# MobilePerceptionLab/EventCalib

Hardware: AMD Instinct MI355X
Metric: Mevents/s DBSCAN+detect (higher is better)
Workload: dtype f64; 1 GPU; ONE 50M-event synthetic circle-grid stream (BASELINE configs[2]'s stream), 346x260, 1 Mev/s, tiled 1.5 ms windows (33334 windows), eps 4 minpts 2; stages: window bounds + EventFrame slicing (reference point order) + DBSCAN(+/-) + circle candidates (reference tie picks); HBM-resident when the timed region starts, upload excluded (reported beside: h2d, ingest); events_total=50000000, events_covered_by_the_ranks_windows=50000000, windows_total=33334, events_per_gpu=50000000, windows_per_gpu=33334, unique_points_per_gpu=38558159, max_window_events=1501, max_segment_points=666, windows_reaching_pairing=26228, circle_candidates=839094, event_point=False

## Files before the change

eventcalib_amd/csrc/extract_window.hpp:

```cpp
#pragma once
#include "ecal_ctx.hpp"
#include "block_utils.hpp"
#include "ref_nth_element.hpp"
#include <type_traits>

#pragma clang fp contract(off)

namespace ecal {

#ifdef ECAL_PHASE_PROF
static __device__ unsigned long long g_det_cycles[16];
#define DET_MARK(idx)                                                                    \
    do {                                                                                 \
        if (threadIdx.x == 0) {                                                          \
            const unsigned long long now__ = __builtin_readcyclecounter();               \
            atomicAdd(&g_det_cycles[idx], now__ - det_t__);                              \
            det_t__ = now__;                                                             \
        }                                                                                \
    } while (0)
#define DET_T0() unsigned long long det_t__ = __builtin_readcyclecounter()
#else
#define DET_MARK(idx) do { } while (0)
#define DET_T0() do { } while (0)
#endif
#ifndef ECAL_DET_STOP
#define ECAL_DET_STOP 0
#endif

constexpr int DET_T = 256;
constexpr uint32_t DET_MAXC = 2048;
constexpr uint32_t DET_LDS_PTS = 1408;
constexpr uint32_t DET_LDS_MAXC = 384;
constexpr uint32_t DET_LDS_PTS2 = 2816, DET_LDS_MAXC2 = 512;

struct DetectParams {
    uint32_t cluster_min;
    uint32_t need_clusters;
    double four_thr2;
    double thr;
    uint32_t fit_circle;
    uint32_t knn;
    const uint32_t *xy16;
    const uint32_t *seg_fmt;
    const uint32_t *px_tree = nullptr, *px_tree_flag = nullptr;
    uint32_t px_tree_epoch = 0;
    int tie_e2i = 0, tie_prune = 0;
};
constexpr uint32_t DET_TIE_TREE_CAP = 768;
constexpr size_t DET_TIE_INV_BYTES = DET_TIE_TREE_CAP;
constexpr uint32_t DET_KNN_MAX = 8;

__device__ __forceinline__ double norm_of(double2 p) { return __dsqrt_rn(p.x * p.x + p.y * p.y); }

struct DetGlobal {
    const double2 *pts;
    uint32_t *members, *sorted, *koff, *ksize, *rep;
    int32_t *kept;
    double *norms;
    __device__ __forceinline__ double2 pt(uint32_t li) const { return pts[li]; }
    __device__ __forceinline__ double norm(uint32_t li) const { return norms[li]; }
    __device__ __forceinline__ double key(uint32_t li) const { return norms[li]; }
    __device__ __forceinline__ void set_norm(uint32_t li, double v) const { norms[li] = v; }
    static constexpr bool INT_PIXELS = false;
    static constexpr uint32_t REP_TIE = 0x80000000u;
    static constexpr uint32_t REP_BAD = 0x40000000u;
    static constexpr uint32_t IDX_MASK = 0xFFFFFFFFu, IDXB = 0u;
    static constexpr int J = 1;
    static constexpr uint32_t MAXC = 0;
    using CIdx = uint32_t;
    static constexpr CIdx CNONE = 0xFFFFFFFFu;
    __device__ __forceinline__ bool composite() const { return false; }
    __device__ __forceinline__ uint32_t member_word(uint32_t, uint32_t i) const { return i; }
    __device__ __forceinline__ uint32_t ipt(uint32_t) const { return 0; }
    __device__ __forceinline__ int32_t label(uint32_t, const int32_t *lab, uint32_t i) const { return lab[i]; }
};
template <uint32_t PTS_, uint32_t MAXC_>
struct DetLdsT {
    static constexpr uint32_t IDXB = PTS_ > 2048u ? 12u : 11u;
    static constexpr uint32_t IDX_MASK = (1u << IDXB) - 1u;
    static constexpr uint32_t REP_TIE = 0x8000u;
    static constexpr uint32_t REP_BAD = 0x4000u;
    static constexpr int J = (int) ((PTS_ + 255u) / 256u);
    static constexpr uint32_t MAXC = MAXC_;
    uint32_t *pts;
    uint32_t *members;
    uint16_t *sorted, *koff, *ksize, *rep;
    int16_t *kept;
    bool small;
    static constexpr bool INT_PIXELS = true;
    using CIdx = uint16_t;
    static constexpr CIdx CNONE = 0xFFFFu;
    __device__ __forceinline__ bool composite() const { return small; }
    __device__ __forceinline__ uint32_t member_word(uint32_t li, uint32_t i) const { return small ? (key(li) << IDXB) | i : i; }
    __device__ __forceinline__ uint32_t ipt(uint32_t li) const { return pts[li]; }
    __device__ __forceinline__ int32_t label(uint32_t li, const int32_t *, uint32_t) const { return kept[li]; }
    __device__ __forceinline__ double2 pt(uint32_t li) const {
        const uint32_t w = pts[li];
        return make_double2((double) (int) (short) (w & 0xFFFFu), (double) (((int) w) >> 16));
    }
    __device__ __forceinline__ double norm(uint32_t li) const { return norm_of(pt(li)); }
    __device__ __forceinline__ uint32_t key(uint32_t li) const {
        const uint32_t w = pts[li];
        const int x = (int) (short) (w & 0xFFFFu), y = ((int) w) >> 16;
        return (uint32_t) (x * x + y * y);
    }
    __device__ __forceinline__ void set_norm(uint32_t, double) const {}
};

struct CircleFit {
    double err, radius, cx, cy;
};

template <typename ST>
__device__ __forceinline__ CircleFit fit_pair(const ST &st, const uint32_t (&base)[2], const uint32_t (&kb)[2], uint32_t kp,
                                              uint32_t kn, double thr) {
    double sx = 0, sy = 0, sxx = 0, syy = 0, sxy = 0, sxxx = 0, syyy = 0, sxyy = 0, sxxy = 0;
    uint32_t cnt = 0;
    for (int pol = 0; pol < 2; pol++) {
        const uint32_t o = base[pol], kk = pol ? kn : kp;
        const uint32_t m = st.ksize[kb[pol] + kk], first = o + st.koff[kb[pol] + kk];
        for (uint32_t t = 0; t < m; t++) {
            const double2 e = st.pt(o + st.sorted[first + t]);
            sx += e.x;
            sy += e.y;
            const double xx = e.x * e.x, yy = e.y * e.y, xy = e.x * e.y;
            sxx += xx;
            syy += yy;
            sxy += xy;
            sxxx += xx * e.x;
            syyy += yy * e.y;
            sxyy += xy * e.y;
            sxxy += e.x * xy;
        }
        cnt += m;
    }
    double A[3][4] = {{2 * sx, 2 * sy, (double) cnt, sxx + syy},
                      {2 * sxx, 2 * sxy, sx, sxxx + sxyy},
                      {2 * sxy, 2 * syy, sy, sxxy + syyy}};
#pragma unroll
    for (int c = 0; c < 3; c++) {
        int piv = c;
#pragma unroll
        for (int r = c + 1; r < 3; r++)
            if (fabs(A[r][c]) > fabs(A[piv][c])) piv = r;
#pragma unroll
        for (int k = 0; k < 4; k++) {
            const double a = A[c][k], b = A[piv][k];
            A[c][k] = b;
            A[piv][k] = (piv == c) ? b : a;
        }
#pragma unroll
        for (int r = c + 1; r < 3; r++) {
            const double f = A[r][c] / A[c][c];
#pragma unroll
            for (int k = c; k < 4; k++) A[r][k] -= f * A[c][k];
        }
    }
    double x[3];
    x[2] = A[2][3] / A[2][2];
    x[1] = (A[1][3] - A[1][2] * x[2]) / A[1][1];
    x[0] = (A[0][3] - A[0][1] * x[1] - A[0][2] * x[2]) / A[0][0];
    CircleFit f;
    f.cx = x[0];
    f.cy = x[1];
    f.radius = __dsqrt_rn(x[0] * x[0] + x[1] * x[1] + x[2]);
    f.err = 0.0;
    const double2 pr = st.pt(base[0] + st.rep[kb[0] + kp]), nr = st.pt(base[1] + st.rep[kb[1] + kn]);
    const double ax = pr.x - nr.x, ay = pr.y - nr.y;
    const double approx = __dsqrt_rn(ax * ax + ay * ay) / 2;
    if (f.radius > thr || f.radius > 2 * approx) {
        f.err = 1.79769313486231570e308;
        return f;
    }
    for (int pol = 0; pol < 2; pol++) {
        const uint32_t o = base[pol], kk = pol ? kn : kp;
        const uint32_t m = st.ksize[kb[pol] + kk], first = o + st.koff[kb[pol] + kk];
        for (uint32_t t = 0; t < m; t++) {
            const double2 e = st.pt(o + st.sorted[first + t]);
            const double ex = e.x - f.cx, ey = e.y - f.cy;
            f.err += fabs(__dsqrt_rn(ex * ex + ey * ey) - f.radius);
        }
    }
    f.err /= (double) cnt * f.radius;
    return f;
}

template <typename ST>
__device__ __forceinline__ uint32_t knn_gated(const ST &st, uint32_t base_pol, uint32_t kb_pol, uint32_t nk, double2 q, uint32_t K,
                                              double gate, uint32_t (&idx)[DET_KNN_MAX]) {
    double d2[DET_KNN_MAX];
    for (uint32_t i = 0; i < DET_KNN_MAX; i++) {
        d2[i] = 1.79769313486231570e308;
        idx[i] = 0;
    }
    uint32_t have = 0;
    for (uint32_t k = 0; k < nk; k++) {
        const double2 c = st.pt(base_pol + st.rep[kb_pol + k]);
        const double dx = q.x - c.x, dy = q.y - c.y;
        const double d = dx * dx + dy * dy;
        uint32_t pos = have < K ? have : K;
        while (pos > 0 && d < d2[pos - 1]) pos--;
        if (pos < K) {
            for (uint32_t m = (have < K ? have : K - 1); m > pos; m--) {
                d2[m] = d2[m - 1];
                idx[m] = idx[m - 1];
            }
            d2[pos] = d;
            idx[pos] = k;
            if (have < K) have++;
        }
    }
    uint32_t real = K;
    for (uint32_t oi = 0; oi < K; oi++)
        if (d2[oi] > d2[0] * 4 || d2[oi] > gate) {
            real = oi;
            break;
        }
    return real;
}

template <typename ST>
__device__ __forceinline__ uint32_t ref_nth_member(const ST &st, uint32_t o, uint32_t *a, uint32_t m, uint32_t nth) {
    ecal::ref_nth_element(a, m, nth, [&](uint32_t x, uint32_t y) { return st.key(o + x) < st.key(o + y); });
    return a[nth];
}

struct LaneArr {
    using value_type = uint32_t;
    uint32_t *v;
    uint32_t off;
    struct Ref {
        uint32_t *v;
        uint32_t lane;
        __device__ __forceinline__ operator uint32_t() const { return (uint32_t) __builtin_amdgcn_readlane((int) *v, (int) lane); }
        __device__ __forceinline__ Ref &operator=(uint32_t x) {
            *v = (threadIdx.x & 63u) == lane ? x : *v;
            return *this;
        }
        __device__ __forceinline__ Ref &operator=(const Ref &o) { return *this = (uint32_t) o; }
    };
    __device__ __forceinline__ Ref operator[](int64_t i) const { return Ref{v, (uint32_t) __builtin_amdgcn_readfirstlane((int) (off + (uint32_t) i))}; }
    __device__ __forceinline__ LaneArr operator+(uint32_t d) const { return LaneArr{v, off + d}; }
};

template <typename ST>
__device__ __forceinline__ bool resolve_ties_inline(const ST &st, const uint32_t (&base)[2], const uint32_t (&kb)[2], const uint32_t (&n_pol)[2],
                                                    const uint32_t (&nk)[2], uint32_t tied0, uint32_t tied1, const uint32_t *tree_win,
                                                    int e2i, int prune, uint32_t *tree_lds, unsigned char *scratch,
                                                    uint8_t *inv, uint32_t *fail_word) {
    constexpr uint32_t WS = 1408, LIST_OFF = 200, LIST_BYTES = WS - LIST_OFF, NIL = 0xFFFFu;
    const uint32_t tid = threadIdx.x, lane = tid & 63u, wave = tid >> 6;
    unsigned char *const ws = scratch + wave * WS;
    uint8_t *const queue = ws + 128;
    uint32_t *const inq = reinterpret_cast<uint32_t *>(ws + 192);
    uint8_t *const lists = ws + LIST_OFF;
    if (tid == 0) *fail_word = 0;
    for (int pol = 0; pol < 2; pol++) {
        __syncthreads();
        if (!(pol ? tied1 : tied0)) continue;
        const uint32_t o = base[pol];
#ifdef ECAL_PHASE_PROF
        const unsigned long long tie_t0__ = __builtin_readcyclecounter();
#endif
        for (uint32_t i = tid; i < n_pol[pol]; i += DET_T) tree_lds[i] = tree_win[o + i];
        __syncthreads();
#ifdef ECAL_PHASE_PROF
        if (tid == 0) atomicAdd(&g_det_cycles[9], __builtin_readcyclecounter() - tie_t0__);
#endif
        for (uint32_t k = wave; k < nk[pol]; k += DET_T / 64) {
            const uint32_t rv = st.rep[kb[pol] + k];
            if (!(rv & ST::REP_TIE)) continue;
            const uint32_t m = st.ksize[kb[pol] + k], first = o + st.koff[kb[pol] + k];
            if (m > 64u || !st.composite()) {
                if (lane == 0) *fail_word = 1;
                continue;
            }
#ifdef ECAL_PHASE_PROF
            unsigned long long tie_t__ = __builtin_readcyclecounter();
#define TIE_MARK(i) do { if (lane == 0) { const unsigned long long n__ = __builtin_readcyclecounter(); atomicAdd(&g_det_cycles[i], n__ - tie_t__); tie_t__ = n__; } } while (0)
            if (lane == 0) {
                atomicAdd(&g_det_cycles[13], 1ull);
                atomicAdd(&g_det_cycles[14], (unsigned long long) m);
            }
#else
#define TIE_MARK(i) do { } while (0)
#endif
            const uint32_t slot = LIST_BYTES / m > 63u ? 63u : LIST_BYTES / m;
            const uint32_t p = lane < m ? st.sorted[first + lane] : 0u;
            if (lane < m) inv[p] = (uint8_t) lane;
            if (lane < 2u) inq[lane] = lane == 0 ? 1u : 0u;
            if (lane == 0) queue[0] = 0;
            __builtin_amdgcn_fence(__ATOMIC_RELEASE, "wavefront");
            __builtin_amdgcn_wave_barrier();
            const bool tiny = m <= 16u;
            unsigned long long hl = 0;
            uint32_t cnt = 0;
            bool bad = false;
            if (lane < m) {
                const uint32_t pw = st.ipt(o + p);
                const int qx = (int) (short) (pw & 0xFFFFu), qy = ((int) pw) >> 16;
                uint8_t *const out = lists + lane * slot;
                unsigned long long s0 = 0, s1 = 0, s2 = 0;
                uint32_t sp = 0, node = 0, dir = 0;
                for (;;) {
                    while (node != NIL) {
                        const uint32_t nw = st.ipt(o + node);
                        const int nx = (int) (short) (nw & 0xFFFFu), ny = ((int) nw) >> 16;
                        const int ddx = nx - qx, ddy = ny - qy;
                        if (ddx * ddx + ddy * ddy <= e2i && node != p && st.kept[o + node] == (int) k) {
                            if (tiny) hl |= (unsigned long long) inv[node] << (4u * cnt);
                            else if (cnt < slot) out[cnt] = inv[node];
                            cnt++;
                        }
                        const int dx = dir ? (qy - ny) : (qx - nx);
                        const uint32_t t = tree_lds[node], l = t & 0xFFFFu, r = t >> 16;
                        const uint32_t nearc = dx <= 0 ? l : r, farc = dx <= 0 ? r : l;
                        if ((dx < 0 ? -dx : dx) <= prune && farc != NIL) {
                            if (sp < 12u) {
                                s2 = (s2 << 16) | (s1 >> 48);
                                s1 = (s1 << 16) | (s0 >> 48);
                                s0 = (s0 << 16) | (farc | ((dir ^ 1u) << 15));
                            }
                            sp++;
                        }
                        node = nearc;
                        dir ^= 1u;
                    }
                    if (sp == 0 || sp > 12u) break;
                    sp--;
                    const uint32_t e = (uint32_t) (s0 & 0xFFFFu);
                    s0 = (s0 >> 16) | (s1 << 48);
                    s1 = (s1 >> 16) | (s2 << 48);
                    s2 >>= 16;
                    node = e & 0x7FFFu;
                    dir = e >> 15;
                }
                bad = (!tiny && cnt > slot) || sp > 12u;
            }
            __builtin_amdgcn_fence(__ATOMIC_RELEASE, "wavefront");
            __builtin_amdgcn_wave_barrier();
            TIE_MARK(10);
            uint32_t head = 0, tail = 1;
            const bool any_bad = __any(bad);
            unsigned long long qv = 0;
            if (tiny && !any_bad) {
                uint32_t inqm = 1u;
                while (head < tail) {
                    const int q = __builtin_amdgcn_readfirstlane((int) ((qv >> (4u * head)) & 15u));
                    head++;
                    const uint32_t lo = (uint32_t) __builtin_amdgcn_readlane((int) (uint32_t) hl, q);
                    const uint32_t hi = (uint32_t) __builtin_amdgcn_readlane((int) (uint32_t) (hl >> 32), q);
                    const unsigned long long hq = ((unsigned long long) hi << 32) | lo;
                    const uint32_t mq = (uint32_t) __builtin_amdgcn_readlane((int) cnt, q);
                    for (uint32_t t = mq; t-- > 0;) {
                        const uint32_t j = (uint32_t) (hq >> (4u * t)) & 15u;
                        if (!((inqm >> j) & 1u)) {
                            inqm |= 1u << j;
                            qv |= (unsigned long long) j << (4u * tail);
                            tail++;
                        }
                    }
                }
            }
            while (!tiny && !any_bad && head < tail) {
                const uint32_t q = reinterpret_cast<volatile uint8_t *>(queue)[head];
                head++;
                const uint32_t mq = (uint32_t) __shfl((int) cnt, (int) q, 64);
                bool take = false;
                uint32_t j = 0;
                if (lane < mq) {
                    j = lists[q * slot + (mq - 1u - lane)];
                    const uint32_t bit = 1u << (j & 31u);
                    take = !(atomicOr(&inq[j >> 5], bit) & bit);
                }
                const unsigned long long mask = __ballot(take);
                if (take) queue[tail + __popcll(mask & ((1ull << lane) - 1ull))] = (uint8_t) j;
                tail += (uint32_t) __popcll(mask);
                __builtin_amdgcn_fence(__ATOMIC_RELEASE, "wavefront");
                __builtin_amdgcn_wave_barrier();
            }
            if (any_bad || tail != m) {
                if (lane == 0) *fail_word = 1;
                continue;
            }
            TIE_MARK(11);
            uint32_t aw = 0;
            if (lane < m) {
                const uint32_t pid = st.sorted[first + (tiny ? (uint32_t) (qv >> (4u * lane)) & 15u : (uint32_t) queue[lane])];
                aw = st.member_word(o + pid, pid);
            }
            ecal::ref_nth_element(LaneArr{&aw, 0u}, m, m / 2u, [](uint32_t x, uint32_t y) { return (x >> ST::IDXB) < (y >> ST::IDXB); });
            const uint32_t pick = (uint32_t) __builtin_amdgcn_readlane((int) aw, (int) (m / 2u)) & ST::IDX_MASK;
            if (lane == 0)
                st.rep[kb[pol] + k] = (typename std::remove_reference<decltype(st.rep[0])>::type) (pick | ST::REP_TIE | ST::REP_BAD);
            TIE_MARK(12);
#undef TIE_MARK
        }
    }
    __syncthreads();
    return *fail_word == 0;
}

template <bool FIT, bool ORD, bool TDET, typename ST>
__device__ __forceinline__ void extract_window(const ST &st, const uint32_t (&base)[2], const uint32_t (&kb)[2],
                                               const uint32_t (&n_pol)[2], const int32_t *lab0, const int32_t *lab1,
                                               const int32_t *ord0, const int32_t *ord1, uint32_t *tie_list, uint32_t *tie_count,
                                               uint32_t tie_token, int32_t *mark0, int32_t *mark1,
                                               const uint32_t (&nc_pol)[2], const DetectParams &prm, uint32_t *csize,
                                               typename ST::CIdx *newid, typename ST::CIdx *coff,
                                               unsigned long long *red, uint32_t *nk_sh, uint32_t *info,
                                               uint32_t *cand_pair, double *cand_xyr, const uint32_t *tie_tree, const uint32_t *tie_flags,
                                               uint8_t *tie_inv) {
    const uint32_t tid = threadIdx.x;
    DET_T0();
    for (int pol = 0; pol < 2; pol++) {
        const uint32_t o = base[pol], ko = kb[pol], n = n_pol[pol], nc = nc_pol[pol];
        const int32_t *lab = pol ? lab1 : lab0;
        for (uint32_t c = tid; c < nc; c += DET_T) csize[c] = 0;
        __syncthreads();
        for (uint32_t i = tid; i < n; i += DET_T) {
            const int32_t l = st.label(o + i, lab, i);
            if (l >= 0) atomicAdd(&csize[l], 1u);
        }
        __syncthreads();
        {
            const uint32_t per = (nc + DET_T - 1) / DET_T, c0 = tid * per;
            uint32_t k = 0, m = 0;
            for (uint32_t c = c0; c < c0 + per && c < nc; c++) {
                if (csize[c] >= prm.cluster_min) {
                    k++;
                    m += csize[c];
                }
            }
            uint32_t ek, em, tk, tm;
            if constexpr (ST::INT_PIXELS) block_exscan_pair16<DET_T>(k, m, red, &ek, &em, &tk, &tm);
            else block_exscan_pair<DET_T>(k, m, red, &ek, &em, &tk, &tm);
            for (uint32_t c = c0; c < c0 + per && c < nc; c++) {
                if (csize[c] >= prm.cluster_min) {
                    newid[c] = (typename ST::CIdx) ek;
                    coff[c] = (typename ST::CIdx) em;
                    st.koff[ko + ek] = em;
                    st.ksize[ko + ek] = csize[c];
                    ek++;
                    em += csize[c];
                } else {
                    newid[c] = ST::CNONE;
                }
            }
            if (tid == 0) {
                nk_sh[pol] = tk;
                nk_sh[2 + pol] = tm;
            }
        }
        __syncthreads();
        for (uint32_t i = tid; i < n; i += DET_T) {
            const int32_t l = st.label(o + i, lab, i);
            int32_t kl = -1;
            if (l >= 0 && newid[l] != ST::CNONE) {
                kl = (int32_t) newid[l];
                const uint32_t at = atomicSub(&csize[l], 1u) - 1u;
                st.members[o + coff[l] + at] = st.member_word(o + i, i);
                st.set_norm(o + i, norm_of(st.pt(o + i)));
            }
            st.kept[o + i] = kl;
        }
        __syncthreads();
    }
    DET_MARK(1);
    if (ECAL_DET_STOP == 2) return;
    const uint32_t nk[2] = {nk_sh[0], nk_sh[1]};
    if (nk[0] < prm.need_clusters || nk[1] < prm.need_clusters) {
        if (tid == 0) {
            info[0] = 0;
            info[1] = nk[0];
            info[2] = nk[1];
            info[3] = 1;
        }
        return;
    }
    const uint32_t tm0 = nk_sh[2], tm1 = nk_sh[3];
    for (uint32_t idx = tid; idx < tm0 + tm1; idx += DET_T) {
        const int pol = idx >= tm0 ? 1 : 0;
        const uint32_t o = base[pol];
        const uint32_t wq = st.members[o + idx - (pol ? tm0 : 0u)];
        const uint32_t i = st.composite() ? (wq & ST::IDX_MASK) : wq;
        const int32_t kl = st.kept[o + i];
        const uint32_t m = st.ksize[kb[pol] + kl], first = o + st.koff[kb[pol] + kl];
        uint32_t rank = 0, at = 0, eq = 0;
        if (st.composite()) {
            const uint32_t wi = wq;
            for (uint32_t t = 0; t < m; t++) {
                const uint32_t wj = st.members[first + t];
                rank += (wj < wi) ? 1u : 0u;
                at += ((wj & ST::IDX_MASK) < i) ? 1u : 0u;
                if constexpr (ORD || TDET) eq += ((wj >> ST::IDXB) == (wi >> ST::IDXB)) ? 1u : 0u;
            }
        } else {
            const auto ni = st.key(o + i);
            for (uint32_t t = 0; t < m; t++) {
                const uint32_t j = st.members[first + t];
                const auto nj = st.key(o + j);
                rank += (nj < ni || (nj == ni && j < i)) ? 1u : 0u;
                at += (j < i) ? 1u : 0u;
                if constexpr (ORD || TDET) eq += (nj == ni) ? 1u : 0u;
            }
        }
        if (rank == m / 2) st.rep[kb[pol] + kl] = ((ORD || TDET) && eq > 1u) ? (i | ST::REP_TIE) : i;
        st.sorted[first + at] = i;
    }
    __syncthreads();
    if constexpr (TDET && !ORD) {
        for (int pol = 0; pol < 2; pol++)
            for (uint32_t k = tid; k < nk[pol]; k += DET_T)
                if (st.rep[kb[pol] + k] & ST::REP_TIE) nk_sh[pol] |= 0x80000000u;
        __syncthreads();
        const uint32_t tied0 = nk_sh[0] >> 31, tied1 = nk_sh[1] >> 31;
        const bool window_tied = (tied0 | tied1) != 0;
        __syncthreads();
        if (tid == 0) {
            nk_sh[0] &= 0x7FFFFFFFu;
            nk_sh[1] &= 0x7FFFFFFFu;
        }
        bool resolved = false;
        if constexpr (ST::INT_PIXELS) {
            if (window_tied && tie_tree) {
                constexpr bool FIRST_LAYOUT = ST::IDXB == 11u;
                constexpr uint32_t TREE_CAP = FIRST_LAYOUT ? DET_TIE_TREE_CAP : 1408u;
                static_assert(FIRST_LAYOUT ? 8u * ST::MAXC >= 4u * DET_TIE_TREE_CAP : 8u * ST::MAXC >= 1408u, "the tree / the positions fit where csize, newid and coff lay");
                uint32_t *const tree_lds = FIRST_LAYOUT ? csize : st.members + 1408;
                uint8_t *const inv = FIRST_LAYOUT ? tie_inv : reinterpret_cast<uint8_t *>(csize);
                const bool ok0 = !tied0 || (n_pol[0] <= TREE_CAP && tie_flags[0] == prm.px_tree_epoch);
                const bool ok1 = !tied1 || (n_pol[1] <= TREE_CAP && tie_flags[1] == prm.px_tree_epoch);
                if (ok0 && ok1 && inv)
                    resolved = resolve_ties_inline(st, base, kb, n_pol, nk, tied0, tied1, tie_tree, prm.tie_e2i, prm.tie_prune, tree_lds,
                                                   reinterpret_cast<unsigned char *>(st.members), inv, &nk_sh[2]);
            }
        }
        for (int pol = 0; pol < 2; pol++)
            for (uint32_t k = tid; k < nk[pol]; k += DET_T) {
                const uint32_t rv = st.rep[kb[pol] + k];
                if (!(rv & ST::REP_TIE)) continue;
                const uint32_t idx = rv & ~(ST::REP_TIE | ST::REP_BAD);
                if (resolved) {
                    st.rep[kb[pol] + k] = idx;
                } else {
                    st.rep[kb[pol] + k] = idx;
                    int32_t *mk = pol ? mark1 : mark0;
                    if (mk) mk[idx] = -3;
                }
            }
        __syncthreads();
        if (tid == 0 && window_tied && !resolved) {
            if (tie_list) tie_list[atomicAdd(tie_count, 1u)] = tie_token | ((tied0 ^ 1u) << 30) | ((tied1 ^ 1u) << 31);
        }
        __syncthreads();
        if (window_tied && !resolved && tie_list) return;
    }
    if constexpr (ORD) {
        if (tid == 0) nk_sh[2] = 0;
        for (int pol = 0; pol < 2; pol++) {
            const int32_t *ord = pol ? ord1 : ord0;
            for (uint32_t i = tid; i < n_pol[pol]; i += DET_T) {
                const int32_t kl = st.kept[base[pol] + i];
                if (kl < 0) continue;
                const uint32_t rv = st.rep[kb[pol] + kl];
                if (!(rv & ST::REP_TIE)) continue;
                const int32_t p = ord ? ord[i] : -1;
                if (p < 0 || (uint32_t) p >= st.ksize[kb[pol] + kl]) st.rep[kb[pol] + kl] = rv | ST::REP_BAD;
            }
        }
        __syncthreads();
        for (int pol = 0; pol < 2; pol++) {
            const int32_t *ord = pol ? ord1 : ord0;
            for (uint32_t i = tid; i < n_pol[pol]; i += DET_T) {
                const int32_t kl = st.kept[base[pol] + i];
                if (kl < 0) continue;
                const uint32_t rv = st.rep[kb[pol] + kl];
                if ((rv & (ST::REP_TIE | ST::REP_BAD)) != ST::REP_TIE) continue;
                st.members[base[pol] + st.koff[kb[pol] + kl] + (uint32_t) ord[i]] = i;
            }
        }
        __syncthreads();
        for (int pol = 0; pol < 2; pol++) {
            for (uint32_t k = tid; k < nk[pol]; k += DET_T) {
                const uint32_t rv = st.rep[kb[pol] + k];
                if (!(rv & ST::REP_TIE)) continue;
                uint32_t pick = rv & ~(ST::REP_TIE | ST::REP_BAD);
                const uint32_t m = st.ksize[kb[pol] + k], first = base[pol] + st.koff[kb[pol] + k];
                if (!(rv & ST::REP_BAD)) pick = ref_nth_member(st, base[pol], &st.members[first], m, m / 2u);
                else nk_sh[2] = 1;
                st.rep[kb[pol] + k] = pick;
            }
        }
        __syncthreads();
    }
    DET_MARK(2);
    if (ECAL_DET_STOP == 3) return;
    uint32_t carry = 0;
    auto emit = [&](uint32_t pi, bool ok, uint32_t ni_best, double cx, double cy, double r) {
        uint32_t ex, dummy, tot, dummy2;
        block_exscan_pair16<DET_T>(ok ? 1u : 0u, 0u, red, &ex, &dummy, &tot, &dummy2);
        if (ok) {
            const size_t at = (size_t) carry + ex;
            cand_pair[2 * at] = pi;
            cand_pair[2 * at + 1] = ni_best;
            cand_xyr[3 * at] = cx;
            cand_xyr[3 * at + 1] = cy;
            cand_xyr[3 * at + 2] = r;
        }
        carry += tot;
    };
    bool paired = false;
    if constexpr (!FIT && ST::INT_PIXELS) {
        if (st.composite() && nk[0] <= 64u && nk[1] <= 64u) {
            paired = true;
            static_assert(4 * ST::MAXC >= 64 * 3 * sizeof(double), "the pair circles take the place of csize[]");
            double *const circ = reinterpret_cast<double *>(csize);
            typename ST::CIdx *const pair_p = newid, *const pair_n = coff;
            double *const term = reinterpret_cast<double *>(st.members);
            uint32_t *const rp = st.members;
            for (uint32_t k = tid; k < nk[0]; k += DET_T) {
                pair_p[k] = ST::CNONE;
                rp[k] = st.ipt(base[0] + st.rep[kb[0] + k]);
            }
            for (uint32_t k = tid; k < nk[1]; k += DET_T) {
                pair_n[k] = ST::CNONE;
                rp[64 + k] = st.ipt(base[1] + st.rep[kb[1] + k]);
            }
            __syncthreads();
            const uint32_t pi = tid;
            bool cand = false;
            uint32_t ni_best = 0;
            double cx = 0, cy = 0, r = 0;
            if (pi < nk[0]) {
                const uint32_t pw = rp[pi];
                const int px = (int) (short) (pw & 0xFFFFu), py = ((int) pw) >> 16;
                uint32_t bi = 0xFFFFFFFFu;
                for (uint32_t k = 0; k < nk[1]; k++) {
                    const uint32_t cw = rp[64 + k];
                    const int dx = px - (int) (short) (cw & 0xFFFFu), dy = py - (((int) cw) >> 16);
                    const uint32_t d = (uint32_t) (dx * dx) + (uint32_t) (dy * dy);
                    if (d < bi) {
                        bi = d;
                        ni_best = k;
                    }
                }
                if (bi != 0xFFFFFFFFu && !((double) bi > prm.four_thr2)) {
                    const uint32_t nw = rp[64 + ni_best];
                    const int nx = (int) (short) (nw & 0xFFFFu), ny = ((int) nw) >> 16;
                    uint32_t bi2 = 0xFFFFFFFFu, back = 0;
                    for (uint32_t k = 0; k < nk[0]; k++) {
                        const uint32_t cw = rp[k];
                        const int dx = nx - (int) (short) (cw & 0xFFFFu), dy = ny - (((int) cw) >> 16);
                        const uint32_t d = (uint32_t) (dx * dx) + (uint32_t) (dy * dy);
                        if (d < bi2) {
                            bi2 = d;
                            back = k;
                        }
                    }
                    if (back == pi) {
                        cand = true;
                        const double2 pc = st.pt(base[0] + st.rep[kb[0] + pi]), nc = st.pt(base[1] + st.rep[kb[1] + ni_best]);
                        cx = (pc.x + nc.x) / 2;
                        cy = (pc.y + nc.y) / 2;
                        const double ddx = pc.x - nc.x, ddy = pc.y - nc.y;
                        r = __dsqrt_rn(ddx * ddx + ddy * ddy) / 2;
                        circ[3 * pi] = cx;
                        circ[3 * pi + 1] = cy;
                        circ[3 * pi + 2] = r;
                        pair_p[pi] = (typename ST::CIdx) pi;
                        pair_n[ni_best] = (typename ST::CIdx) pi;
                    }
                }
            }
            __syncthreads();
            constexpr int J = ST::J;
            const uint32_t n_all = n_pol[0] + n_pol[1];
            double tv[J];
#pragma unroll
            for (int j = 0; j < J; j++) {
                const uint32_t li = tid + j * DET_T;
                tv[j] = 0.0;
                if (li < n_all) {
                    const int pol = li >= n_pol[0] ? 1 : 0;
                    const int32_t kl = st.kept[li];
                    if (kl >= 0) {
                        const uint32_t pr = pol ? pair_n[kl] : pair_p[kl];
                        if (pr != ST::CNONE) {
                            const double2 e = st.pt(li);
                            const double ex = e.x - circ[3 * pr], ey = e.y - circ[3 * pr + 1];
                            tv[j] = fabs(__dsqrt_rn(ex * ex + ey * ey) - circ[3 * pr + 2]);
                        }
                    }
                }
            }
            __syncthreads();
#pragma unroll
            for (int j = 0; j < J; j++) {
                const uint32_t li = tid + j * DET_T;
                if (li < n_all) term[li] = tv[j];
            }
            __syncthreads();
            bool ok = false;
            if (cand) {
                double fit = 0;
                uint32_t cnt = 0;
                for (int pol = 0; pol < 2; pol++) {
                    const uint32_t o = base[pol], kk = pol ? ni_best : pi;
                    const uint32_t m = st.ksize[kb[pol] + kk], first = o + st.koff[kb[pol] + kk];
                    for (uint32_t t = 0; t < m; t++) fit += term[o + st.sorted[first + t]];
                    cnt += m;
                }
                fit /= (double) cnt * r;
                ok = fit < 10 / r;
            }
            emit(pi, ok, ni_best, cx, cy, r);
        }
    }
    for (uint32_t p0 = 0; !paired && p0 < nk[0]; p0 += DET_T) {
        const uint32_t pi = p0 + tid;
        bool ok = false;
        uint32_t ni_best = 0;
        double cx = 0, cy = 0, r = 0;
        if (FIT && pi < nk[0]) {
            uint32_t n_idx[DET_KNN_MAX], p_idx[DET_KNN_MAX];
            uint32_t real = knn_gated(st, base[1], kb[1], nk[1], st.pt(base[0] + st.rep[kb[0] + pi]), prm.knn, prm.four_thr2,
                                      n_idx);
            if (real > 0) {
                CircleFit best = fit_pair(st, base, kb, pi, n_idx[0], prm.thr);
                uint32_t nmin = 0;
                for (uint32_t j = 1; j < real; j++) {
                    const CircleFit f = fit_pair(st, base, kb, pi, n_idx[j], prm.thr);
                    if (f.err < best.err) {
                        best = f;
                        nmin = j;
                    }
                }
                if (best.err < 2 / best.radius) {
                    const uint32_t nsel = n_idx[nmin];
                    real = knn_gated(st, base[0], kb[0], nk[0], st.pt(base[1] + st.rep[kb[1] + nsel]), prm.knn, prm.four_thr2,
                                     p_idx);
                    if (real > 0) {
                        CircleFit bb = fit_pair(st, base, kb, p_idx[0], nsel, prm.thr);
                        uint32_t pmin = 0;
                        for (uint32_t i = 1; i < real; i++) {
                            const CircleFit f = fit_pair(st, base, kb, p_idx[i], nsel, prm.thr);
                            if (f.err < bb.err) {
                                bb = f;
                                pmin = i;
                            }
                        }
                        if (p_idx[pmin] == pi) {
                            ok = true;
                            ni_best = nsel;
                            cx = bb.cx;
                            cy = bb.cy;
                            r = bb.radius;
                        }
                    }
                }
            }
        } else if (pi < nk[0]) {
            const double2 pc = st.pt(base[0] + st.rep[kb[0] + pi]);
            double bd = 1.79769313486231570e308;
            uint32_t back = 0;
            bool near = false;
            bool int_nn = false;
            if constexpr (ST::INT_PIXELS) int_nn = st.composite();
            if (int_nn) {
                const uint32_t pw = st.ipt(base[0] + st.rep[kb[0] + pi]);
                const int px = (int) (short) (pw & 0xFFFFu), py = ((int) pw) >> 16;
                uint32_t bi = 0xFFFFFFFFu;
                for (uint32_t k = 0; k < nk[1]; k++) {
                    const uint32_t cw = st.ipt(base[1] + st.rep[kb[1] + k]);
                    const int dx = px - (int) (short) (cw & 0xFFFFu), dy = py - (((int) cw) >> 16);
                    const uint32_t d = (uint32_t) (dx * dx) + (uint32_t) (dy * dy);
                    if (d < bi) {
                        bi = d;
                        ni_best = k;
                    }
                }
                if (bi != 0xFFFFFFFFu) bd = (double) bi;
                if (!(bd > prm.four_thr2)) {
                    near = true;
                    const uint32_t nw = st.ipt(base[1] + st.rep[kb[1] + ni_best]);
                    const int nx = (int) (short) (nw & 0xFFFFu), ny = ((int) nw) >> 16;
                    uint32_t bi2 = 0xFFFFFFFFu;
                    for (uint32_t k = 0; k < nk[0]; k++) {
                        const uint32_t cw = st.ipt(base[0] + st.rep[kb[0] + k]);
                        const int dx = nx - (int) (short) (cw & 0xFFFFu), dy = ny - (((int) cw) >> 16);
                        const uint32_t d = (uint32_t) (dx * dx) + (uint32_t) (dy * dy);
                        if (d < bi2) {
                            bi2 = d;
                            back = k;
                        }
                    }
                }
            } else {
                for (uint32_t k = 0; k < nk[1]; k++) {
                    const double2 c = st.pt(base[1] + st.rep[kb[1] + k]);
                    const double dx = pc.x - c.x, dy = pc.y - c.y;
                    const double d = dx * dx + dy * dy;
                    if (d < bd) {
                        bd = d;
                        ni_best = k;
                    }
                }
                if (!(bd > prm.four_thr2)) {
                    near = true;
                    const double2 nc = st.pt(base[1] + st.rep[kb[1] + ni_best]);
                    double bd2 = 1.79769313486231570e308;
                    for (uint32_t k = 0; k < nk[0]; k++) {
                        const double2 c = st.pt(base[0] + st.rep[kb[0] + k]);
                        const double dx = nc.x - c.x, dy = nc.y - c.y;
                        const double d = dx * dx + dy * dy;
                        if (d < bd2) {
                            bd2 = d;
                            back = k;
                        }
                    }
                }
            }
            if (near) {
                const double2 nc = st.pt(base[1] + st.rep[kb[1] + ni_best]);
                if (back == pi) {
                    cx = (pc.x + nc.x) / 2;
                    cy = (pc.y + nc.y) / 2;
                    const double ddx = pc.x - nc.x, ddy = pc.y - nc.y;
                    r = __dsqrt_rn(ddx * ddx + ddy * ddy) / 2;
                    double fit = 0;
                    uint32_t cnt = 0;
                    for (int pol = 0; pol < 2; pol++) {
                        const uint32_t o = base[pol], kk = pol ? ni_best : pi;
                        const uint32_t m = st.ksize[kb[pol] + kk], first = o + st.koff[kb[pol] + kk];
                        for (uint32_t t = 0; t < m; t++) {
                            const double2 e = st.pt(o + st.sorted[first + t]);
                            const double ex = e.x - cx, ey = e.y - cy;
                            fit += fabs(__dsqrt_rn(ex * ex + ey * ey) - r);
                        }
                        cnt += m;
                    }
                    fit /= (double) cnt * r;
                    ok = fit < 10 / r;
                }
            }
        }
        emit(pi, ok, ni_best, cx, cy, r);
    }
    DET_MARK(3);
    if (tid == 0) {
        info[0] = carry;
        info[1] = nk[0];
        info[2] = nk[1];
        info[3] = (ORD && nk_sh[2]) ? ECAL_WIN_TIE_FALLBACK : 0u;
    }
}

template <uint32_t PTS, uint32_t MAXC>
struct DetLdsLayoutT {
    static constexpr size_t csize_off = 0;
    static constexpr size_t newid_off = csize_off + 4 * MAXC;
    static constexpr size_t coff_off = newid_off + 2 * MAXC;
    static constexpr size_t koff_off = coff_off + 2 * MAXC;
    static constexpr size_t ksize_off = koff_off + 4 * MAXC;
    static constexpr size_t rep_off = ksize_off + 4 * MAXC;
    static constexpr size_t sorted_off = rep_off + 4 * MAXC;
    static constexpr size_t kept_off = sorted_off + 2 * PTS;
    static constexpr size_t members_off = kept_off + 2 * PTS;
    static constexpr size_t pts_off = members_off + 4 * PTS;
    static constexpr size_t bytes = pts_off + 4 * PTS;
};

template <bool FIT, uint32_t PTS, uint32_t MAXC, bool FIRST, bool KNOWN = false, bool ORD = false, bool TDET = false>
__device__ __forceinline__ void extract_one(
    unsigned char *smem, unsigned long long *red, uint32_t *nk_sh, const uint32_t s, const double *__restrict__ xy,
    const uint32_t *__restrict__ seg_off, const uint32_t *__restrict__ seg_cnt, const int32_t *__restrict__ labels,
    const uint32_t *__restrict__ n_clusters, const DetectParams &prm, uint32_t *__restrict__ win_info,
    uint32_t *__restrict__ cand_pair, double *__restrict__ cand_xyr, int32_t *__restrict__ kept_labels,
    uint32_t *__restrict__ rep, uint32_t *__restrict__ members, uint32_t *__restrict__ koff, uint32_t *__restrict__ ksize,
    uint32_t *__restrict__ sorted, double *__restrict__ norms, uint32_t *__restrict__ todo, uint32_t *__restrict__ todo_count,
    const uint32_t *known = nullptr, const int32_t *__restrict__ order = nullptr, uint32_t *tie_list = nullptr,
    uint32_t *tie_count = nullptr, int32_t *tie_mark = nullptr) {
    using LL = DetLdsLayoutT<PTS, MAXC>;
    const uint32_t tid = threadIdx.x;
    const double2 *pts = reinterpret_cast<const double2 *>(xy);
    uint32_t *info = win_info + 4 * (size_t) s;
    const uint32_t o_pol[2] = {KNOWN ? known[0] : seg_off[2 * s], KNOWN ? known[1] : seg_off[2 * s + 1]};
    const uint32_t n_pol[2] = {KNOWN ? known[2] : seg_cnt[2 * s], KNOWN ? known[3] : seg_cnt[2 * s + 1]};
    const uint32_t nc_pol[2] = {KNOWN ? known[4] : n_clusters[2 * s], KNOWN ? known[5] : n_clusters[2 * s + 1]};

    if (n_pol[0] == 0 || n_pol[1] == 0 || nc_pol[0] > DET_MAXC || nc_pol[1] > DET_MAXC) {
        for (int pol = 0; pol < 2; pol++)
            for (uint32_t i = tid; i < n_pol[pol]; i += DET_T) kept_labels[o_pol[pol] + i] = -1;
        if (tid == 0) {
            info[0] = 0;
            info[1] = 0;
            info[2] = 0;
            info[3] = (n_pol[0] == 0 || n_pol[1] == 0) ? 1 : 4;
        }
        return;
    }
    const bool contiguous = o_pol[1] == o_pol[0] + n_pol[0];
    const uint32_t n_all = n_pol[0] + n_pol[1];
    bool staged = contiguous && n_all <= PTS && nc_pol[0] <= MAXC && nc_pol[1] <= MAXC;
    if (FIRST && !staged && contiguous && n_all <= DET_LDS_PTS2 && nc_pol[0] <= DET_LDS_MAXC2 && nc_pol[1] <= DET_LDS_MAXC2 && todo) {
        if (tid == 0) todo[atomicAdd(todo_count, 1u)] = s;
        return;
    }
    uint32_t *csize = reinterpret_cast<uint32_t *>(smem);
    uint32_t *const lds_pts = reinterpret_cast<uint32_t *>(smem + LL::pts_off);
    DET_T0();
    bool small_px = false;
    constexpr double KEY_LIM = PTS > 2048u ? 723.0 : 1023.0;
    if (staged) {
        bool fits = true, large = false;
        constexpr int JS = (int) ((PTS + DET_T - 1) / DET_T);
        const bool packed = !KNOWN && prm.xy16 && (prm.seg_fmt[2 * s] & 1u);
        double2 vin[JS];
        uint32_t win[JS];
        int32_t lin[JS];
#pragma unroll
        for (int j = 0; j < JS; j++) {
            const uint32_t i = min(tid + j * DET_T, n_all - 1u);
            if (packed) win[j] = prm.xy16[o_pol[0] + i];
            else vin[j] = pts[o_pol[0] + i];
            lin[j] = labels[o_pol[0] + i];
        }
#pragma unroll
        for (int j = 0; j < JS; j++) {
            const uint32_t i = tid + j * DET_T;
            if (i < n_all) {
                double2 v;
                if (packed) v = make_double2((double) (int) (short) (win[j] & 0xFFFFu), (double) (((int) win[j]) >> 16));
                else v = vin[j];
                fits = fits && v.x == floor(v.x) && v.y == floor(v.y) && fabs(v.x) <= 32767.0 && fabs(v.y) <= 32767.0;
                large = large || !(fabs(v.x) <= KEY_LIM && fabs(v.y) <= KEY_LIM);
                lds_pts[i] = ((uint32_t) (int) v.x & 0xFFFFu) | ((uint32_t) (int) v.y << 16);
                reinterpret_cast<int16_t *>(smem + LL::kept_off)[i] = (int16_t) lin[j];
            }
        }
        if (tid == 0) nk_sh[0] = 0;
        __syncthreads();
        if (!fits || large) atomicOr(&nk_sh[0], (fits ? 0u : 1u) | (large ? 2u : 0u));
        __syncthreads();
        const uint32_t verdict = nk_sh[0];
        staged = !(verdict & 1);
        small_px = !(verdict & 2);
        DET_MARK(0);
        if (ECAL_DET_STOP == 1) {
            for (uint32_t i = tid; i < n_all; i += DET_T) kept_labels[o_pol[0] + i] = (int32_t) lds_pts[i];
            return;
        }
    }
    if (staged) {
        DetLdsT<PTS, MAXC> st;
        st.sorted = reinterpret_cast<uint16_t *>(smem + LL::sorted_off);
        st.koff = reinterpret_cast<uint16_t *>(smem + LL::koff_off);
        st.ksize = reinterpret_cast<uint16_t *>(smem + LL::ksize_off);
        st.rep = reinterpret_cast<uint16_t *>(smem + LL::rep_off);
        st.kept = reinterpret_cast<int16_t *>(smem + LL::kept_off);
        st.members = reinterpret_cast<uint32_t *>(smem + LL::members_off);
        st.pts = lds_pts;
        st.small = small_px;
        const uint32_t base[2] = {0u, n_pol[0]};
        const uint32_t kb[2] = {0u, MAXC};
        uint8_t *tie_inv = nullptr;
        const uint32_t *tie_tree = nullptr, *tie_flags = nullptr;
        if constexpr (TDET && !KNOWN) {
            if (prm.px_tree) {
                if constexpr (FIRST) tie_inv = smem + (LL::bytes > 3 * DET_MAXC * sizeof(uint32_t) ? LL::bytes : 3 * DET_MAXC * sizeof(uint32_t));
                tie_tree = prm.px_tree + o_pol[0];
                tie_flags = prm.px_tree_flag + 2 * (size_t) s;
            }
        }
        extract_window<FIT, ORD, TDET>(st, base, kb, n_pol, labels + o_pol[0], labels + o_pol[1], order ? order + o_pol[0] : nullptr,
                                       order ? order + o_pol[1] : nullptr, tie_list, tie_count, s, tie_mark ? tie_mark + o_pol[0] : nullptr,
                                       tie_mark ? tie_mark + o_pol[1] : nullptr, nc_pol, prm, csize,
                       reinterpret_cast<uint16_t *>(smem + LL::newid_off), reinterpret_cast<uint16_t *>(smem + LL::coff_off), red, nk_sh, info, cand_pair + 2 * (size_t) o_pol[0],
                       cand_xyr + 3 * (size_t) o_pol[0], tie_tree, tie_flags, tie_inv);
        __syncthreads();
#ifdef ECAL_PHASE_PROF
        det_t__ = __builtin_readcyclecounter();
#endif
        for (uint32_t i = tid; i < n_all; i += DET_T) kept_labels[o_pol[0] + i] = st.kept[i];
        if (nk_sh[0] >= prm.need_clusters && nk_sh[1] >= prm.need_clusters) {
            for (int pol = 0; pol < 2; pol++)
                for (uint32_t k = tid; k < nk_sh[pol]; k += DET_T) rep[o_pol[pol] + k] = st.rep[kb[pol] + k];
        }
        DET_MARK(4);
        if (tid == 0) {
#ifdef ECAL_PHASE_PROF
            atomicAdd(&g_det_cycles[8], 1ull);
#endif
        }
    } else {
        DetGlobal st;
        const uint32_t w0 = o_pol[0] < o_pol[1] ? o_pol[0] : o_pol[1];
        st.pts = pts + w0;
        st.members = members + w0;
        st.sorted = sorted + w0;
        st.koff = koff + w0;
        st.ksize = ksize + w0;
        st.rep = rep + w0;
        st.kept = kept_labels + w0;
        st.norms = norms + w0;
        const uint32_t base[2] = {o_pol[0] - w0, o_pol[1] - w0};
        extract_window<FIT, ORD, TDET>(st, base, base, n_pol, labels + o_pol[0], labels + o_pol[1], order ? order + o_pol[0] : nullptr,
                                       order ? order + o_pol[1] : nullptr, tie_list, tie_count, s, tie_mark ? tie_mark + o_pol[0] : nullptr,
                                       tie_mark ? tie_mark + o_pol[1] : nullptr, nc_pol, prm, csize, csize + DET_MAXC,
                       csize + 2 * DET_MAXC, red, nk_sh, info, cand_pair + 2 * (size_t) o_pol[0],
                       cand_xyr + 3 * (size_t) o_pol[0], nullptr, nullptr, nullptr);
    }
}
constexpr size_t DET_LDS_BYTES_GLOBAL = 3 * DET_MAXC * sizeof(uint32_t);
constexpr size_t DET_LDS_BYTES_STAGED = DetLdsLayoutT<DET_LDS_PTS, DET_LDS_MAXC>::bytes;
static_assert(DET_LDS_BYTES_STAGED + DET_TIE_INV_BYTES + 64 <= 26624, "six workgroups per CU");
constexpr size_t DET_LDS_BYTES2 = DetLdsLayoutT<DET_LDS_PTS2, DET_LDS_MAXC2>::bytes > DET_LDS_BYTES_GLOBAL
                                      ? DetLdsLayoutT<DET_LDS_PTS2, DET_LDS_MAXC2>::bytes : DET_LDS_BYTES_GLOBAL;
constexpr size_t DET_LDS_BYTES = DET_LDS_BYTES_STAGED > DET_LDS_BYTES_GLOBAL ? DET_LDS_BYTES_STAGED : DET_LDS_BYTES_GLOBAL;

}
```

Baseline: 21200 Mevents/s.

## Spread mutual-nearest-neighbor pairing across all waves with packed atomicMin

The composite pairing path previously had one thread per positive cluster scan every negative cluster, then do a second scan back to check the match was mutual. Now each of the four waves takes a slice of the negative clusters. It packs (squared distance << 6 | index) into one word and uses LDS atomicMin to fill row-best and column-best tables in a single pass, which gives both directions with the same lowest-index tie rule. Candidate emission is replaced by a single-wave ballot/popcount compaction instead of the generic emit lambda. The cost is extra LDS atomics and a dependence on members[] having room for the two extra 64-entry tables. The new emit assumes the output starts at offset zero and sets carry only in the first wave.

```diff
diff --git a/eventcalib_amd/csrc/extract_window.hpp b/eventcalib_amd/csrc/extract_window.hpp
--- a/eventcalib_amd/csrc/extract_window.hpp
+++ b/eventcalib_amd/csrc/extract_window.hpp
@@ -619,13 +619,38 @@
             typename ST::CIdx *const pair_p = newid, *const pair_n = coff;
             double *const term = reinterpret_cast<double *>(st.members);
             uint32_t *const rp = st.members;
+            static_assert(2u * 2046u * 2046u < (1u << 26), "d << 6 | index fits 32 bits and never is the all-ones word");
+            static_assert(ST::J >= 1, "members[] holds rp[128], rowbest[64] and colbest[64]");
+            uint32_t *const rowbest = st.members + 128, *const colbest = st.members + 192;
             for (uint32_t k = tid; k < nk[0]; k += DET_T) {
                 pair_p[k] = ST::CNONE;
                 rp[k] = st.ipt(base[0] + st.rep[kb[0] + k]);
+                rowbest[k] = 0xFFFFFFFFu;
             }
             for (uint32_t k = tid; k < nk[1]; k += DET_T) {
                 pair_n[k] = ST::CNONE;
                 rp[64 + k] = st.ipt(base[1] + st.rep[kb[1] + k]);
+                colbest[k] = 0xFFFFFFFFu;
+            }
+            __syncthreads();
+            {
+                const uint32_t lane = tid & 63u, wave = (uint32_t) __builtin_amdgcn_readfirstlane((int) (tid >> 6));
+                const uint32_t cq = (nk[1] + 3u) >> 2, j0 = wave * cq, j1 = min(j0 + cq, nk[1]);
+                if (lane < nk[0] && j0 < j1) {
+                    const uint32_t pw = rp[lane];
+                    const int px = (int) (short) (pw & 0xFFFFu), py = ((int) pw) >> 16;
+                    uint32_t k = (lane + j0) % nk[1], cwd = rp[64 + k], best = 0xFFFFFFFFu;
+                    for (uint32_t j = j0; j < j1; j++) {
+                        const uint32_t kn = k + 1u == nk[1] ? 0u : k + 1u, nxt = rp[64 + kn];
+                        const int dx = px - (int) (short) (cwd & 0xFFFFu), dy = py - (((int) cwd) >> 16);
+                        const uint32_t d = (uint32_t) (dx * dx) + (uint32_t) (dy * dy);
+                        best = min(best, (d << 6) | k);
+                        atomicMin(&colbest[k], (d << 6) | lane);
+                        k = kn;
+                        cwd = nxt;
+                    }
+                    atomicMin(&rowbest[lane], best);
+                }
             }
             __syncthreads();
             const uint32_t pi = tid;
@@ -633,31 +658,10 @@
             uint32_t ni_best = 0;
             double cx = 0, cy = 0, r = 0;
             if (pi < nk[0]) {
-                const uint32_t pw = rp[pi];
-                const int px = (int) (short) (pw & 0xFFFFu), py = ((int) pw) >> 16;
-                uint32_t bi = 0xFFFFFFFFu;
-                for (uint32_t k = 0; k < nk[1]; k++) {
-                    const uint32_t cw = rp[64 + k];
-                    const int dx = px - (int) (short) (cw & 0xFFFFu), dy = py - (((int) cw) >> 16);
-                    const uint32_t d = (uint32_t) (dx * dx) + (uint32_t) (dy * dy);
-                    if (d < bi) {
-                        bi = d;
-                        ni_best = k;
-                    }
-                }
-                if (bi != 0xFFFFFFFFu && !((double) bi > prm.four_thr2)) {
-                    const uint32_t nw = rp[64 + ni_best];
-                    const int nx = (int) (short) (nw & 0xFFFFu), ny = ((int) nw) >> 16;
-                    uint32_t bi2 = 0xFFFFFFFFu, back = 0;
-                    for (uint32_t k = 0; k < nk[0]; k++) {
-                        const uint32_t cw = rp[k];
-                        const int dx = nx - (int) (short) (cw & 0xFFFFu), dy = ny - (((int) cw) >> 16);
-                        const uint32_t d = (uint32_t) (dx * dx) + (uint32_t) (dy * dy);
-                        if (d < bi2) {
-                            bi2 = d;
-                            back = k;
-                        }
-                    }
+                const uint32_t rb = rowbest[pi], bi = rb >> 6;
+                ni_best = rb & 63u;
+                if (rb != 0xFFFFFFFFu && !((double) bi > prm.four_thr2)) {
+                    const uint32_t back = colbest[ni_best] & 63u;
                     if (back == pi) {
                         cand = true;
                         const double2 pc = st.pt(base[0] + st.rep[kb[0] + pi]), nc = st.pt(base[1] + st.rep[kb[1] + ni_best]);
@@ -714,7 +718,18 @@
                 fit /= (double) cnt * r;
                 ok = fit < 10 / r;
             }
-            emit(pi, ok, ni_best, cx, cy, r);
+            if (tid < 64u) {
+                const unsigned long long okm = __ballot(ok);
+                if (ok) {
+                    const size_t at = (size_t) __popcll(okm & ((1ull << tid) - 1ull));
+                    cand_pair[2 * at] = pi;
+                    cand_pair[2 * at + 1] = ni_best;
+                    cand_xyr[3 * at] = cx;
+                    cand_xyr[3 * at + 1] = cy;
+                    cand_xyr[3 * at + 2] = r;
+                }
+                carry = (uint32_t) __popcll(okm);
+            }
         }
     }
     for (uint32_t p0 = 0; !paired && p0 < nk[0]; p0 += DET_T) {
```

Result: no change. 21380 Mevents/s, median of 6 (+0.8%).
